# ORNL/DDStore

Measured on NVIDIA H100. Metric: batch_fetch_GBps, higher is better.
Workload: dtype u8

## Files before the change

### ddstore_b200/csrc/kernels.cu

```cuda
#include <cuda_runtime.h>
#include <stdint.h>
#include <stdio.h>
#include <stdlib.h>
#include <string.h>

#include <algorithm>
#include <atomic>
#include <type_traits>

#include "kernels.h"

namespace {

thread_local char g_cuda_err[512] = "";
std::atomic<unsigned long long> g_launches{0};

#define CUDA_TRY(expr)                                                                                   \
    do {                                                                                                 \
        cudaError_t e__ = (expr);                                                                        \
        if (e__ != cudaSuccess) {                                                                        \
            snprintf(g_cuda_err, sizeof(g_cuda_err), "%s failed: %s (%s:%d)", #expr, cudaGetErrorString(e__), \
                     __FILE__, __LINE__);                                                                \
            return (int)e__ ? (int)e__ : -1;                                                             \
        }                                                                                                \
// ... 1004 lines not shown
    return T;
}

struct PieceDesc {
    int64_t dpos;
    uint32_t n, pack;
};

__device__ __forceinline__ void spin_until_done(const unsigned int *ovl, unsigned int q, unsigned long long *status,
                                                unsigned long long tag, int64_t nreq) {
    const uint64_t t0 = globaltimer_ns();
    while ((int)(ld_acquire_u32(&ovl[4 + (q & 3u)]) - q) < 0) {
        __nanosleep(100);
        if (globaltimer_ns() - t0 > 4000000000ull) {
            report(status, tag, nreq, DDSK_CODE_WATCHDOG);
            __trap();
        }
    }
}

template <bool FIXED, int NW, int S, int CH, int PCAP, bool CVT = false, bool NORM = false, bool PAD = false, bool PUT = false>
__global__ void __launch_bounds__(NW * 32, 1) dds_gather_kernel(const __grid_constant__ GatherArgs a,
                                                                const __grid_constant__ CvtParam<CVT> c) {
    static_assert(CVT || !NORM, "a normalising launch is a converting one");
    static_assert(FIXED || !PAD, "a padded batch is a fixed-stride walk");
    static_assert(!PUT || (!CVT && !PAD), "a put writes raw rows");
    constexpr int STAGE = CH + 32;
    constexpr bool PUSH = FIXED && !CVT && !PAD && !PUT;
    extern __shared__ __align__(128) unsigned char smem_dyn[];
    __shared__ __align__(8) uint64_t full_bar[NW][S];
    __shared__ __align__(16) PieceDesc desc[NW][S][32];
    __shared__ int64_t wtot[PCAP > 0 ? NW : 1];
    __shared__ int64_t push_rbase[PUSH ? DDSK_MAX_RANKS + 1 : 1];
    __shared__ uint64_t push_win[PUSH ? DDSK_MAX_RANKS : 1];

    const int lane = threadIdx.x & 31;
    const int warp = threadIdx.x >> 5;
    const int64_t gwarp = (int64_t)blockIdx.x * NW + warp;
    const int64_t nwarps = (int64_t)gridDim.x * NW;

    if (lane == 0) {
#pragma unroll
        for (int s = 0; s < S; s++) mbar_init(smem_u32(&full_bar[warp][s]), 1);
        fence_mbar_init();
    }
    uint32_t lut_s = 0;
    if constexpr (CVT) {
        lut_s = smem_u32(smem_dyn) + (uint32_t)(NW * S * STAGE + (PCAP ? PCAP * 12 + 16 : 0));
        for (int i = threadIdx.x; i < c.lut_bytes / 4; i += NW * 32) sts32(lut_s + 4u * (uint32_t)i, c.lut[i]);
        __syncthreads();
    }
    int code0 = 0;
    if constexpr (CVT) code0 = c.code[0];
    if (a.dbg && threadIdx.x == 0) a.dbg[blockIdx.x * 4 + 0] = globaltimer_ns();
    if (a.overlap && !a.wait1_valid) {
        asm volatile("griddepcontrol.wait;" ::: "memory");
        asm volatile("griddepcontrol.launch_dependents;" ::: "memory");
    } else {
        asm volatile("griddepcontrol.launch_dependents;" ::: "memory");
        if (!a.skip_wait) asm volatile("griddepcontrol.wait;" ::: "memory");
    }
    bool gate_open = !(a.overlap && a.wait2_valid);
    auto pass_gate = [&]() {
        if (!gate_open) {
            if (lane == 0) spin_until_done(a.ovl, a.seq - 2u, a.status, a.status_tag, a.nreq);
            __syncwarp();
            gate_open = true;
        }
    };

    ChunkWalker<FIXED, CH, PCAP, CVT, PAD, PUT> w;
    if (!FIXED) {
        if constexpr (PCAP > 0) {
            w.pv.src_s = smem_u32(smem_dyn) + (uint32_t)(NW * S * STAGE);
            w.pv.dst_s = w.pv.src_s + (uint32_t)PCAP * 8u;
            const bool writer = blockIdx.x == 0;
            if (writer) pass_gate();
            w.T = plan_in_smem<NW, PCAP, CVT, NORM, PUT>(a, w.pv, wtot, warp, lane, writer, code0);
        } else {
            w.pv.src = a.req_src;
            w.pv.dst = a.req_dst;
            w.pv.seg_tab = a.seg_tab;
            if (a.wait_plan) {
                const bool need_gate = !gate_open;
                unsigned long long pw = 0;
                const uint64_t t0 = globaltimer_ns();
                while (true) {
                    bool ok = true;
                    if (lane == 0) {
                        pw = ld_acquire_u64(&a.plan_word[a.seq & 3u]);
                        ok = (pw >> 40) == (unsigned long long)a.plan_tiles;
                    } else if (lane == 1 && need_gate) {
                        ok = (int)(ld_acquire_u32(&a.ovl[4 + ((a.seq - 2u) & 3u)]) - (a.seq - 2u)) >= 0;
                    }
                    if (__all_sync(0xffffffffu, ok)) break;
                    __nanosleep(100);
                    if (globaltimer_ns() - t0 > 4000000000ull) {
                        report(a.status, a.status_tag, a.nreq, DDSK_CODE_WATCHDOG);
                        __trap();
                    }
                }
                gate_open = true;
                w.T = (int64_t)(__shfl_sync(0xffffffffu, pw, 0) & 0xFFFFFFFFFFull);
            } else {
                w.T = __ldcg(&a.req_dst[a.nreq]);
            }
        }
    }

    const bool push = PUSH && a.push != nullptr;
    if (FIXED && push) {
        const ddsk_push_t *ps = a.push;
        const int P = ps->nranks, me = ps->me, par = (int)(a.push_step & 1ull);
        if (blockIdx.x == 0 && threadIdx.x == 0) {
            unsigned long long *hdr = (unsigned long long *)ps->win[me];
            *(volatile unsigned long long *)&hdr[1 + par] = (unsigned long long)a.push_nreq;
            __threadfence_system();
            st_release_sys_u64(&hdr[0], a.push_step);
        }
        const uint64_t t0 = globaltimer_ns();
        for (int r0 = 0; r0 < P; r0 += 32) {
            const int r = r0 + lane;
            while (r < P && ld_acquire_sys_u64((const unsigned long long *)ps->win[r]) < a.push_step) {
                __nanosleep(200);
                if (globaltimer_ns() - t0 > 30000000000ull) {
                    report(a.status, a.status_tag, a.nreq, DDSK_CODE_WATCHDOG);
                    __trap();
                }
            }
        }
        __syncwarp();
        if (warp == 0) {
            int64_t n = 0;
            for (int r0 = 0; r0 < P; r0 += 32) {
                const int r = r0 + lane;
                int64_t mine_n = 0;
                if (r < P) {
                    push_win[r] = (uint64_t)ps->win[r];
                    mine_n = ld_relaxed_sys_s64((const int64_t *)ps->win[r] + 1 + par);
                }
                const int64_t incl = warp_incl_scan(mine_n, lane);
                if (r < P) push_rbase[r] = n + incl - mine_n;
                n += __shfl_sync(0xffffffffu, incl, 31);
            }
            if (lane == 0) push_rbase[P] = n;
        }
        __syncthreads();
        w.push_n = P;
        w.push_me = me;
        w.push_par = par;
        w.push_rbase = push_rbase;
        w.push_win = push_win;
        w.push_idx_off = ps->idx_off[par];
    }
    if (a.dbg && threadIdx.x == 0) a.dbg[blockIdx.x * 4 + 1] = globaltimer_ns();
    bool dbg_first = a.dbg != nullptr && warp == 0;
    w.gwarp = gwarp;
    w.nwarps = nwarps;
    w.static_claims = a.tickets == nullptr;
    w.gate_ok = gate_open;
    if constexpr (PAD) w.nb = a.pad_slot;
    else w.nb = (FIXED && a.count <= a.var.lenlist[a.var.nranks - 1]) ? a.count * a.var.row_bytes : 0;
    w.nreq = (FIXED && push) ? push_rbase[w.push_n] : a.nreq;
    if (FIXED) w.T = w.nb * w.nreq;
    bool over = w.T > a.dst_cap;
    const int64_t push_dst_off = (FIXED && push) ? a.push->dst_off[w.push_par] : 0;
    const bool multi = !FIXED && a.plan.nvars > 1;
    int64_t vbase[DDSK_MAX_MULTI + 1];
#pragma unroll
    for (int v = 0; v <= DDSK_MAX_MULTI; v++) vbase[v] = INT64_MAX;
    if (multi) {
        over = false;
#pragma unroll
        for (int v = 0; v < DDSK_MAX_MULTI; v++)
            if (v < a.plan.nvars) vbase[v] = w.pv.d((int64_t)v * a.plan.per_var);
#pragma unroll
        for (int v = 0; v < DDSK_MAX_MULTI; v++)
            if (v < a.plan.nvars) {
                const int64_t endv = v + 1 < a.plan.nvars ? vbase[v + 1] : w.T;
                over |= endv - vbase[v] > a.mcap[v];
            }
        if (PCAP > 0) over |= w.T > 0xFFFFFFFFll;
        if constexpr (CVT) {
            w.valign = true;
#pragma unroll
            for (int v = 0; v < DDSK_MAX_MULTI; v++) w.vb[v] = vbase[v];
        }
    }
    auto dst_of = [&](int64_t dpos) -> char * {
        if (FIXED && push) {
            int p = 0;
            for (int k = 1; k < w.push_n; k++)
                if (dpos >= push_rbase[k] * w.nb) p = k;
            return (char *)push_win[p] + push_dst_off + (dpos - push_rbase[p] * w.nb);
        }
        if (!multi) return a.dst + dpos;
        int64_t b = vbase[0];
        char *d = a.mdst[0];
#pragma unroll
        for (int k = 1; k < DDSK_MAX_MULTI; k++)
            if (dpos >= vbase[k]) {
                b = vbase[k];
                d = a.mdst[k];
            }
        return d + (dpos - b);
    };
    auto out_of = [&](int64_t dpos, int &code, uint32_t &lut) -> char * {
        if constexpr (CVT) {
            if (!multi) {
// ... 158 lines not shown
        }
        }
        bulk_commit();
        __syncwarp();
        consumed++;
    }
    if (PUT || a.overlap || (FIXED && push)) {
        bulk_wait_all<0>();
        fence_proxy_async_global();
    } else {
        bulk_wait_read<0>();
    }
    __syncwarp();
    pass_gate();
    if (multi) {
        for (int64_t i = gwarp * 32 + lane; i < a.nreq + a.plan.nvars; i += nwarps * 32) {
            const int v = (int)(i / (a.plan.per_var + 1));
            const int64_t j = i - (int64_t)v * (a.plan.per_var + 1);
            if (v < a.plan.nvars && a.moffsets[v]) {
                const int64_t basev = w.pv.d((int64_t)v * a.plan.per_var);
                int64_t e = (v * a.plan.per_var + j == a.nreq) ? w.T : w.pv.d((int64_t)v * a.plan.per_var + j);
                if constexpr (CVT) a.moffsets[v][j] = cvt_scale<NORM>(e - basev, c.code[v]);
                else a.moffsets[v][j] = e - basev;
            }
        }
        if constexpr (CVT) {
            if (gwarp == 0 && lane == 0 && a.total_out) {
                int64_t t = 0;
#pragma unroll
                for (int v = 0; v < DDSK_MAX_MULTI; v++)
                    if (v < a.plan.nvars) t += cvt_scale<NORM>((v + 1 < a.plan.nvars ? vbase[v + 1] : w.T) - vbase[v], c.code[v]);
                *a.total_out = t;
            }
        }
    }
    if constexpr (PAD) {
        if (a.pad_lengths || w.nb == 0) {
            for (int64_t i = gwarp * 32 + lane; i < a.nreq; i += nwarps * 32) {
                uint64_t src;
                int64_t payload;
                pad_lookup(a, i, src, payload);
                if (a.pad_lengths) a.pad_lengths[i] = payload / a.var.row_bytes;
            }
        }
    }
    if (FIXED && a.offsets_out && !push) {
        if constexpr (CVT) {
            for (int64_t i = gwarp * 32 + lane; i <= a.nreq; i += nwarps * 32) a.offsets_out[i] = cvt_scale<NORM>(i * w.nb, code0);
        } else {
            for (int64_t i = gwarp * 32 + lane; i <= a.nreq; i += nwarps * 32) a.offsets_out[i] = i * w.nb;
        }
    }

    if (a.dbg && lane == 0) atomicMax(&a.dbg[blockIdx.x * 4 + 3], (unsigned long long)globaltimer_ns());
    if (a.overlap) {
        if (lane == 0) {
            __threadfence();
            const unsigned int slot = a.seq & 3u;
            const unsigned int done = atomicAdd(&a.ovl[slot], 1u);
            if (done == (unsigned int)(nwarps - 1)) {
                a.ovl[slot] = 0;
                a.ovl[8 + slot] = 0;
                if (a.wait_plan) a.plan_word[slot] = 0;
                if (a.wait1_valid) spin_until_done(a.ovl, a.seq - 1u, a.status, a.status_tag, a.nreq);
                __threadfence();
                st_release_u32(&a.ovl[4 + slot], a.seq);
            }
        }
    } else if (lane == 0) {
        if (FIXED && push) __threadfence_system(); else __threadfence();
        unsigned int done = atomicAdd(&a.counters[1], 1u);
        if (done == (unsigned int)(nwarps - 1)) {
            a.counters[0] = 0;
            a.counters[1] = 0;
            __threadfence();
            if (FIXED && push) {
                const ddsk_push_t *ps = a.push;
                for (int r = 0; r < ps->nranks; r++)
                    st_release_sys_u64((unsigned long long *)ps->win[r] + 8 + ps->me, a.push_step);
                const unsigned long long *hdr = (const unsigned long long *)ps->win[ps->me];
                const uint64_t t0 = globaltimer_ns();
                for (int r = 0; r < ps->nranks; r++)
                    while (ld_acquire_sys_u64(&hdr[8 + r]) < a.push_step) {
                        __nanosleep(200);
                        if (globaltimer_ns() - t0 > 30000000000ull) {
                            report(a.status, a.status_tag, a.nreq, DDSK_CODE_WATCHDOG);
                            __trap();
                        }
                    }
                const unsigned long long st = *(volatile const unsigned long long *)&hdr[3];
                if (st != DDSK_STATUS_OK) atomicMin(a.status, st | a.status_tag);
            }
            if (a.host_mirror) {
                a.host_mirror[0] = *(volatile unsigned long long *)a.status;
                a.host_mirror[1] = (unsigned long long)w.T;
                __threadfence_system();
            }
        }
    }
}

__global__ void __launch_bounds__(256) dds_small_get_kernel(const __grid_constant__ ddsk_var_t var, int64_t start, int64_t count,
                                                            char *__restrict__ dst, int64_t dst_cap,
                                                            volatile unsigned long long *flag, unsigned long long ticket) {
    uint64_t src = 0;
    const int code = dev_locate(var, start, count, &src);
    const int64_t n = code ? 0 : count * var.row_bytes;
    unsigned long long st = DDSK_STATUS_OK;
    if (code) st = (unsigned long long)code;
    else if (n > dst_cap) st = ((unsigned long long)1 << 8) | DDSK_CODE_CAPACITY;
    if (st == DDSK_STATUS_OK && n > 0) {
        const char *s = (const char *)src;
        if ((((uint64_t)s | (uint64_t)dst | (uint64_t)n) & 15u) == 0) {
            const uint4 *s4 = (const uint4 *)s;
            uint4 *d4 = (uint4 *)dst;
            for (int64_t i = threadIdx.x; i < (n >> 4); i += blockDim.x) d4[i] = s4[i];
        } else if ((((uint64_t)s | (uint64_t)dst | (uint64_t)n) & 3u) == 0) {
            const uint32_t *s1 = (const uint32_t *)s;
            uint32_t *d1 = (uint32_t *)dst;
            for (int64_t i = threadIdx.x; i < (n >> 2); i += blockDim.x) d1[i] = s1[i];
        } else {
            for (int64_t i = threadIdx.x; i < n; i += blockDim.x) dst[i] = s[i];
        }
    }
    __threadfence_system();
// ... 215 lines not shown
                for (int64_t i = threadIdx.x; i < (n >> 2); i += blockDim.x) ((uint32_t *)dp)[i] = __ldcg((const unsigned int *)sp + i);
            } else {
                for (int64_t i = threadIdx.x; i < n; i += blockDim.x) dp[i] = __ldcg(sp + i);
            }
            __threadfence_system();
        }
        __syncthreads();
        if (threadIdx.x == 0) *(volatile unsigned long long *)&mb->resp = (q << 8) | st;
        served = q;
    }
}

__global__ void dds_touch_kernel(const uint4 *__restrict__ p, size_t n, unsigned int *sink) {
    unsigned int acc = 0;
    for (size_t i = (size_t)blockIdx.x * blockDim.x + threadIdx.x; i < n; i += (size_t)gridDim.x * blockDim.x) {
        const uint4 v = p[i];
        acc ^= v.x ^ v.y ^ v.z ^ v.w;
    }
    if (acc == 0x9E3779B9u && sink) *sink = acc;
}

__global__ void dds_occupy_kernel(unsigned long long ns, int smem_bytes) {
    extern __shared__ unsigned char occ_smem[];
    if ((int)threadIdx.x < smem_bytes) occ_smem[threadIdx.x] = (unsigned char)threadIdx.x;
    const uint64_t t0 = globaltimer_ns();
    while (globaltimer_ns() - t0 < ns) __nanosleep(1000);
    if ((int)threadIdx.x < smem_bytes && occ_smem[threadIdx.x] == 255 && ns == 0) printf("");
}

struct Geometry {
    int nw, stages, ch, pcap;
};
constexpr Geometry kGeoms[] = {{8, 4, 4096, 0}, {8, 6, 4096, 0}, {16, 3, 4096, 0}, {4, 4, 8192, 0}, {12, 4, 4096, 0}, {4, 6, 4096, 0},
                               {6, 4, 4096, 0},
                               {12, 3, 4096, 0}};
constexpr int kNumGeoms = (int)(sizeof(kGeoms) / sizeof(kGeoms[0]));
constexpr Geometry kGeomsS[] = {{12, 3, 4096, 4096}, {12, 3, 3072, 8192}, {16, 3, 2048, 8192}, {16, 3, 3072, 4096}, {8, 4, 4096, 4096}};
constexpr int kNumGeomsS = (int)(sizeof(kGeomsS) / sizeof(kGeomsS[0]));
constexpr int64_t kPlanSmemMax = 8192;
int64_t g_plan_smem_default = 1024;

constexpr int kGeomLarge = 4, kGeomSmall = 2, kGeomVar = 4;

int g_geom_fixed_env = -1;
int g_geom_var_env = -1;
int g_geom_s_env = -1;
int g_min_seg_var = 4, g_min_seg_s = 2;
bool g_geom_init = false;
int g_sms = 0;
int g_ctas_per_sm = 1;
int g_pdl = 1;
unsigned long long *g_dbg = nullptr;
constexpr size_t kDbgRegion = 4096 + 8;
int g_l2_persist = 1;
int g_smem_plan = 1;

int pick_geometry() {
    if (g_geom_init) return 0;
    int dev = 0;
    CUDA_TRY(cudaGetDevice(&dev));
    CUDA_TRY(cudaDeviceGetAttribute(&g_sms, cudaDevAttrMultiProcessorCount, dev));
    if (const char *e = getenv("DDS_GATHER_GEOM")) g_geom_fixed_env = atoi(e);
    if (g_geom_fixed_env >= kNumGeoms) g_geom_fixed_env = -1;
    g_geom_var_env = g_geom_fixed_env;
    if (const char *e = getenv("DDS_GATHER_GEOM_VAR")) g_geom_var_env = atoi(e);
    if (g_geom_var_env >= kNumGeoms) g_geom_var_env = -1;
    if (const char *e = getenv("DDS_GATHER_GEOM_S")) g_geom_s_env = atoi(e);
    if (g_geom_s_env >= kNumGeomsS) g_geom_s_env = -1;
    if (const char *e = getenv("DDS_VAR_MINSEG")) g_min_seg_var = atoi(e) > 0 ? atoi(e) : 4;
    if (const char *e = getenv("DDS_S_MINSEG")) g_min_seg_s = atoi(e) > 0 ? atoi(e) : 2;
    if (const char *e = getenv("DDS_GATHER_CTAS_PER_SM")) g_ctas_per_sm = atoi(e) > 0 ? atoi(e) : 1;
    if (const char *e = getenv("DDS_PDL")) g_pdl = atoi(e) != 0;
    if (const char *e = getenv("DDS_SMEM_PLAN")) g_smem_plan = atoi(e);
    if (const char *e = getenv("DDS_SMEM_PLAN_MAX")) g_plan_smem_default = atoll(e);
    if (const char *e = getenv("DDS_L2_PERSIST")) g_l2_persist = atoi(e);
    if (const char *e = getenv("DDS_DEBUG_TIMING"))
        if (atoi(e)) {
            CUDA_TRY(cudaMalloc((void **)&g_dbg, 2 * kDbgRegion * 8));
            CUDA_TRY(cudaMemset(g_dbg, 0, 2 * kDbgRegion * 8));
        }
    g_geom_init = true;
    return 0;
}

int geometry_for(bool fixed, int64_t request_bytes) {
    if (fixed) {
        if (g_geom_fixed_env >= 0) return g_geom_fixed_env;
        return request_bytes < 2048 ? kGeomSmall : kGeomLarge;
    }
    return g_geom_var_env >= 0 ? g_geom_var_env : kGeomVar;
}
int geometry_s_for(int64_t nreq) {
    if (nreq > kPlanSmemMax || nreq > g_plan_smem_default) return -1;
    if (g_geom_s_env >= 0 && kGeomsS[g_geom_s_env].pcap >= nreq) return g_geom_s_env;
    return nreq <= 4096 ? 0 : 1;
}

constexpr int smem_bytes_of(int nw, int s, int ch, int pcap) { return nw * s * (ch + 32) + (pcap ? pcap * 12 + 16 : 0); }
int static_smem_of(int nw, int s) { return nw * s * (8 + 32 * 16) + 16 * 8 + 64; }
int ctas_per_sm_for(int nw, int s, int ch, int pcap) {
    int per_sm = g_ctas_per_sm;
    while (per_sm > 1 && per_sm * (smem_bytes_of(nw, s, ch, pcap) + static_smem_of(nw, s) + 1024) > 227 * 1024) per_sm--;
    return per_sm;
}

bool cvt_has_norm(const ddsk_cvt_t *cvt) {
    for (int v = 0; v < DDSK_MAX_MULTI; v++)
        if (DDSK_CVT_IS_NORM(cvt->code[v])) return true;
    return false;
}

template <bool FIXED, int NW, int S, int CH, int PCAP, bool CVT = false, bool NORM = false, bool PAD = false, bool PUT = false>
int launch_gather_t(const GatherArgs &args_in, cudaStream_t stream, const ddsk_cvt_t *cvt = nullptr) {
    const int smem = smem_bytes_of(NW, S, CH, PCAP) + (CVT ? cvt->lut_bytes : 0);
    static std::atomic<unsigned long long> configured{0};
    auto kern = dds_gather_kernel<FIXED, NW, S, CH, PCAP, CVT, NORM, PAD, PUT>;
    int dev = 0;
    CUDA_TRY(cudaGetDevice(&dev));
    if (CVT) {
        if (dev >= 64 || !(configured.load() & (1ull << dev))) {
            cudaFuncAttributes fa;
            int optin = 0;
            CUDA_TRY(cudaFuncGetAttributes(&fa, kern));
            CUDA_TRY(cudaDeviceGetAttribute(&optin, cudaDevAttrMaxSharedMemoryPerBlockOptin, dev));
            const int most = std::min(smem_bytes_of(NW, S, CH, PCAP) + DDSK_MAX_MULTI * 1024, optin - (int)fa.sharedSizeBytes);
            CUDA_TRY(cudaFuncSetAttribute(kern, cudaFuncAttributeMaxDynamicSharedMemorySize, most));
            if (dev < 64) configured.fetch_or(1ull << dev);
        }
    } else if (dev >= 64 || !(configured.load() & (1ull << dev))) {
        CUDA_TRY(cudaFuncSetAttribute(kern, cudaFuncAttributeMaxDynamicSharedMemorySize, smem));
        if (dev < 64) configured.fetch_or(1ull << dev);
    }
    const int per_sm = ctas_per_sm_for(NW, S, CH, PCAP);
    GatherArgs args = args_in;
    args.dbg = g_dbg ? g_dbg + (size_t)(args.overlap ? (args.seq & 1u) : 0u) * kDbgRegion : nullptr;
    cudaLaunchConfig_t cfg = {};
    cfg.gridDim = dim3((unsigned)(g_sms * per_sm));
    cfg.blockDim = dim3(NW * 32);
    cfg.dynamicSmemBytes = smem;
    cfg.stream = stream;
    cudaLaunchAttribute attr[1];
    attr[0].id = cudaLaunchAttributeProgrammaticStreamSerialization;
    attr[0].val.programmaticStreamSerializationAllowed = g_pdl ? 1 : 0;
    cfg.attrs = attr;
    cfg.numAttrs = 1;
    if constexpr (CVT) {
        CUDA_TRY(cudaLaunchKernelEx(&cfg, kern, args, *cvt));
    } else {
        CUDA_TRY(cudaLaunchKernelEx(&cfg, kern, args, NoCvt{0}));
    }
    g_launches++;
    return 0;
}

template <int NW, int S, int CH, int PCAP>
bool cvt_s_fits_t(int lut_bytes) {
    cudaFuncAttributes fa;
    int dev = 0, optin = 0;
    if (cudaGetDevice(&dev) != cudaSuccess || cudaFuncGetAttributes(&fa, dds_gather_kernel<false, NW, S, CH, PCAP, true>) != cudaSuccess ||
        cudaDeviceGetAttribute(&optin, cudaDevAttrMaxSharedMemoryPerBlockOptin, dev) != cudaSuccess) {
        (void)cudaGetLastError();
        return false;
    }
    return smem_bytes_of(NW, S, CH, PCAP) + lut_bytes + (int)fa.sharedSizeBytes <= optin;
}

thread_local const void *g_l2_base = nullptr;
thread_local size_t g_l2_bytes = 0;

template <typename... KArgs, typename... Args>
int launch_pdl(void (*kern)(KArgs...), dim3 grid, dim3 block, cudaStream_t st, Args... args) {
    cudaLaunchConfig_t cfg = {};
    cfg.gridDim = grid;
    cfg.blockDim = block;
    cfg.dynamicSmemBytes = 0;
    cfg.stream = st;
    cudaLaunchAttribute attr[2];
    attr[0].id = cudaLaunchAttributeProgrammaticStreamSerialization;
    attr[0].val.programmaticStreamSerializationAllowed = g_pdl ? 1 : 0;
    cfg.attrs = attr;
    cfg.numAttrs = 1;
    if (g_l2_base && g_l2_bytes && g_l2_persist) {
        attr[1].id = cudaLaunchAttributeAccessPolicyWindow;
        attr[1].val.accessPolicyWindow.base_ptr = const_cast<void *>(g_l2_base);
        attr[1].val.accessPolicyWindow.num_bytes = g_l2_bytes;
        attr[1].val.accessPolicyWindow.hitRatio = 1.0f;
        attr[1].val.accessPolicyWindow.hitProp = cudaAccessPropertyPersisting;
        attr[1].val.accessPolicyWindow.missProp = cudaAccessPropertyStreaming;
        cfg.numAttrs = 2;
    }
    g_l2_base = nullptr;
    g_l2_bytes = 0;
    CUDA_TRY(cudaLaunchKernelEx(&cfg, kern, args...));
    g_launches++;
    return 0;
}

template <bool FIXED>
int launch_gather(const GatherArgs &args, cudaStream_t stream, const ddsk_cvt_t *cvt, bool put = false) {
    if (put) return launch_gather_t<FIXED, 12, 4, 4096, 0, false, false, false, true>(args, stream);
    if (cvt) return cvt_has_norm(cvt) ? launch_gather_t<FIXED, 12, 4, 4096, 0, true, true>(args, stream, cvt)
                                      : launch_gather_t<FIXED, 12, 4, 4096, 0, true>(args, stream, cvt);
    const int64_t request_bytes = args.count < ((int64_t)1 << 20) ? args.count * args.var.row_bytes : INT64_MAX;
    switch (geometry_for(FIXED, FIXED ? request_bytes : 0)) {
    case 1: return launch_gather_t<FIXED, 8, 6, 4096, 0>(args, stream);
    case 2: return launch_gather_t<FIXED, 16, 3, 4096, 0>(args, stream);
    case 3: return launch_gather_t<FIXED, 4, 4, 8192, 0>(args, stream);
    case 4: return launch_gather_t<FIXED, 12, 4, 4096, 0>(args, stream);
    case 5: return launch_gather_t<FIXED, 4, 6, 4096, 0>(args, stream);
    case 6: return launch_gather_t<FIXED, 6, 4, 4096, 0>(args, stream);
    case 7: return launch_gather_t<FIXED, 12, 3, 4096, 0>(args, stream);
    default: return launch_gather_t<FIXED, 8, 4, 4096, 0>(args, stream);
    }
}
int launch_gather_s(int g, const GatherArgs &args, cudaStream_t stream, const ddsk_cvt_t *cvt, bool put) {
    if (put)
        return g == 1 ? launch_gather_t<false, 12, 3, 3072, 8192, false, false, false, true>(args, stream)
                      : launch_gather_t<false, 12, 3, 4096, 4096, false, false, false, true>(args, stream);
    if (cvt && cvt_has_norm(cvt))
        return g == 1 ? launch_gather_t<false, 12, 3, 3072, 8192, true, true>(args, stream, cvt)
                      : launch_gather_t<false, 12, 3, 4096, 4096, true, true>(args, stream, cvt);
    if (cvt) return g == 1 ? launch_gather_t<false, 12, 3, 3072, 8192, true>(args, stream, cvt)
                           : launch_gather_t<false, 12, 3, 4096, 4096, true>(args, stream, cvt);
    switch (g) {
    case 1: return launch_gather_t<false, 12, 3, 3072, 8192>(args, stream);
    case 2: return launch_gather_t<false, 16, 3, 2048, 8192>(args, stream);
    case 3: return launch_gather_t<false, 16, 3, 3072, 4096>(args, stream);
    case 4: return launch_gather_t<false, 8, 4, 4096, 4096>(args, stream);
    default: return launch_gather_t<false, 12, 3, 4096, 4096>(args, stream);
    }
}

int select_s(int64_t nreq, int64_t cap, const ddsk_cvt_t *cvt, bool put = false) {
    if (!g_smem_plan || cap >= ((int64_t)1 << 32)) return -1;
    if (!cvt && !put) return geometry_s_for(nreq);
    if (nreq > kPlanSmemMax || nreq > g_plan_smem_default) return -1;
    if (put) return nreq <= 4096 ? 0 : 1;
    if (nreq <= 4096) return cvt_s_fits_t<12, 3, 4096, 4096>(cvt->lut_bytes) ? 0 : -1;
    return cvt_s_fits_t<12, 3, 3072, 8192>(cvt->lut_bytes) ? 1 : -1;
}

void fill_overlap(GatherArgs &a, const ddsk_scratch_t *scr, int flags) {
    a.overlap = (flags & DDSK_F_OVERLAP) ? 1 : 0;
    a.skip_wait = (flags & DDSK_F_SKIP_WAIT) ? 1 : 0;
    a.wait1_valid = (flags & DDSK_F_PREV1) ? 1 : 0;
    a.wait2_valid = (flags & DDSK_F_PREV2) ? 1 : 0;
    a.seq = scr->ovl_seq;
    a.ovl = scr->ovl;
    a.tickets = a.overlap ? nullptr : scr->counters;
}

}

extern "C" {

const char *ddsk_last_cuda_error(void) { return g_cuda_err; }
// ... 51 lines not shown
    if (int rc = pick_geometry()) return rc;
    GatherArgs a;
    memset(&a, 0, sizeof(a));
    a.var = *var;
    a.count = count;
    a.nreq = nreq;
    a.dst = nullptr;
    a.dst_cap = INT64_MAX;
    a.status = scr->status;
    a.status_tag = scr->status_tag;
    a.counters = scr->counters;
    a.tickets = scr->counters;
    a.min_seg_chunks = 1;
    a.push = push_dev;
    if (nreq > 0)
        CUDA_TRY(cudaMemcpyAsync(push_host->win[push_host->me] + push_host->idx_off[step & 1ull], starts_dev, (size_t)nreq * 8,
                                 cudaMemcpyDeviceToDevice, st));
    a.push_nreq = nreq;
    a.push_step = step;
    return launch_gather<true>(a, st, nullptr);
}

int ddsk_gather_padded(const ddsk_var_t *var, const ddsk_index_t *index, int64_t nreq, int64_t max_rows, uint64_t pad_bits,
                       int pad_log2, int64_t *lengths, void *dst_dev, const ddsk_scratch_t *scr, int flags,
                       const ddsk_cvt_t *cvt, void *stream) {
    cudaStream_t st = (cudaStream_t)stream;
    if (flags & DDSK_F_RESET) CUDA_TRY(cudaMemsetAsync(scr->status, 0xFF, sizeof(unsigned long long), st));
    if (nreq <= 0) return 0;
    if (int rc = pick_geometry()) return rc;
    GatherArgs a;
    memset(&a, 0, sizeof(a));
    a.var = *var;
    a.plan.starts = index->starts;
    a.plan.counts = index->counts;
    a.plan.ids = index->sample_ids;
    a.plan.tab = (const longlong2 *)index->table;
    a.plan.nsamples = index->nsamples;
    a.count = max_rows;
    a.nreq = nreq;
    a.dst = (char *)dst_dev;
    a.pad_slot = max_rows * var->row_bytes;
    a.dst_cap = nreq * a.pad_slot;
    a.pad_bits = pad_bits;
    a.pad_log2 = pad_log2;
    a.pad_in_log2 = cvt ? cvt_in_log2<true>(cvt->code[0]) : 0;
    a.pad_out_log2 = cvt ? cvt_out_log2<true>(cvt->code[0]) : 0;
    a.pad_lengths = lengths;
    a.status = scr->status;
    a.status_tag = scr->status_tag;
    a.counters = scr->counters;
    a.min_seg_chunks = 1;
    fill_overlap(a, scr, flags);
    a.host_mirror = (flags & DDSK_F_MIRROR) ? scr->host_mirror : nullptr;
    if (!cvt) return launch_gather_t<true, 12, 4, 4096, 0, false, false, true>(a, st);
    return cvt_has_norm(cvt) ? launch_gather_t<true, 12, 4, 4096, 0, true, true, true>(a, st, cvt)
                             : launch_gather_t<true, 12, 4, 4096, 0, true, false, true>(a, st, cvt);
}

static int plan_and_gather(const ddsk_var_t *var, const PlanSrc &p, int64_t nreq, int64_t cap_total, GatherArgs &a,
                           int64_t *offsets_dev_or_null, ddsk_scratch_t *scr, int flags, const ddsk_cvt_t *cvt,
                           cudaStream_t st) {
    a.nreq = nreq;
    a.status = scr->status;
    a.status_tag = scr->status_tag;
    a.counters = scr->counters;
    a.host_mirror = (flags & DDSK_F_MIRROR) ? scr->host_mirror : nullptr;
    a.plan = p;
    a.total_out = scr->total;
    const bool put = (flags & DDSK_F_PUT) != 0;
    const int gs = select_s(nreq, cap_total, cvt, put);
    if (gs >= 0) {
        a.offsets_out = offsets_dev_or_null;
        a.min_seg_chunks = g_min_seg_s;
        fill_overlap(a, scr, flags);
        if (a.overlap) a.tickets = scr->ovl + 8 + (a.seq & 3u);
        return launch_gather_s(gs, a, st, cvt, put);
    }
    if (nreq > scr->cap_req || cap_total / SEG_GRAIN + 2 > scr->seg_cap) {
        snprintf(g_cuda_err, sizeof(g_cuda_err), "ddsk_gather_var: scratch too small (%lld requests > %lld, or %lld segments > %lld)",
                 (long long)nreq, (long long)scr->cap_req, (long long)(cap_total / SEG_GRAIN + 2), (long long)scr->seg_cap);
        return -2;
    }
    PlanProto pr;
    memset(&pr, 0, sizeof(pr));
    if (flags & DDSK_F_OVERLAP) {
        pr.dbg = g_dbg ? g_dbg + (size_t)(scr->ovl_seq & 1u) * kDbgRegion : nullptr;
        pr.ovl = scr->ovl;
        pr.plan_word = scr->plan_word;
        pr.seq = scr->ovl_seq;
        pr.skip_wait = (flags & DDSK_F_SKIP_WAIT) ? 1 : 0;
        pr.wait2_valid = (flags & DDSK_F_PREV2) ? 1 : 0;
        pr.wait4_valid = (flags & DDSK_F_PREV4) ? 1 : 0;
    }
    const int tiles = (int)((nreq + PLAN_TILE - 1) / PLAN_TILE);
    scr->plan_tag = (scr->plan_tag + 1) & 0x3FFFFFu;
    if (p.ids && (p.tab || p.mtab[0])) {
        g_l2_base = p.tab ? (const void *)p.tab : (const void *)p.mtab[0];
        g_l2_bytes = (size_t)(p.tab ? p.nsamples : p.mnsamples[0]) * 16;
    }
    if (int rc = launch_pdl(put ? dds_plan_kernel<true> : dds_plan_kernel<false>, dim3(tiles), dim3(PLAN_THREADS), st, *var, p, nreq, scr->req_src, scr->req_dst,
                            (unsigned long long *)scr->tile_sums, scr->plan_tag, offsets_dev_or_null, scr->seg_tab, scr->seg_cap,
                            scr->status, scr->status_tag, pr, cvt && p.nvars <= 1 ? (int)cvt->code[0] : 0))
        return rc;
    a.req_src = scr->req_src;
    a.req_dst = scr->req_dst;
    a.seg_tab = scr->seg_tab;
// ... 155 lines not shown
```

### ddstore_b200/cython/pyddstore.pyx

```
"""pyddstore -- Cython binding with the reference module's name and Python surface
(/root/reference/src/pyddstore.pyx:58-131: PyDDStore(comm, method=0) with add / get / epoch_begin /
epoch_end / free / init / update), bound to the C++ class in include/ddstore_b200.hpp, which is a thin
wrapper over the C-ABI (include/ddstore_b200.h) of libddstore_b200.so.

Differences from the reference binding, all at the edges:
  * `comm` is anything ddstore_b200.comm.as_dds_comm accepts (an mpi4py-style communicator, a
    torch.distributed adapter, ShmComm, None) -- MPI is not required;
  * arrays may also be CUDA tensors / __cuda_array_interface__ objects (then nothing touches the host);
  * `get_batch` fetches a whole batch in one kernel launch.
"""
from libcpp.string cimport string
from libcpp cimport bool as cbool
from libc.stdint cimport uint64_t

import numpy as np

from ddstore_b200.comm import as_dds_comm
from ddstore_b200.store import _Buf, _conversion, _dtype_name, _i64, _norm_tables, _pad_bits, _ptr

cdef extern from *:
    """
    static void dds_translate_exception() {
        try { throw; }
        catch (const std::invalid_argument &e) { PyErr_SetString(PyExc_ValueError, e.what()); }
        catch (const std::out_of_range &e) { PyErr_SetString(PyExc_KeyError, e.what()); }
        catch (const std::exception &e) { PyErr_SetString(PyExc_RuntimeError, e.what()); }
    }
    """
    void dds_translate_exception()

cdef extern from "ddstore_b200.h":
    ctypedef struct dds_comm_t:
        pass

cdef extern from "ddstore_b200.hpp" nogil:
    cdef cppclass DDStore:
        DDStore(int method, dds_comm_t* comm, int device) except +dds_translate_exception
        void add[T](string name, T* buffer, long nrows, int disp) except +dds_translate_exception
        void add_device[T](string name, const T* buffer, long nrows, int disp) except +dds_translate_exception
        void get[T](string name, long start, long count, T* buffer) except +dds_translate_exception
        void get_device[T](string name, long start, long count, T* buffer) except +dds_translate_exception
        long get_batch[T](string name, const long* starts, const long* counts, long fixed_count, long nreq, T* dst,
                          long cap, long* offsets, cbool on_device, void* stream) except +dds_translate_exception
        long get_batch_convert(string name, const long* starts, const long* counts, long fixed_count, long nreq,
                               void* dst, long cap, int code, const void* lut, long* offsets, cbool idx_on_device,
                               void* stream) except +dds_translate_exception
        long get_batch_padded_convert(string name, const long* starts, const long* counts, long nreq, int itemsize,
                                      int code, const void* lut, long max_rows, uint64_t pad_bits, void* dst, long cap,
                                      long* lengths, cbool idx_on_device, void* stream) except +dds_translate_exception
        void set_normalization(string name, const float* mean, const float* std, long nchan, long inner,
                               cbool tables_on_device) except +dds_translate_exception
        long put_batch[T](string name, const long* starts, const long* counts, long fixed_count, long nreq, const T* src,
                          long src_bytes, cbool idx_on_device, void* stream) except +dds_translate_exception
        void epoch_begin() except +dds_translate_exception
        void epoch_end() except +dds_translate_exception
        void free() except +dds_translate_exception
        void init(string name, long nrows, int disp, int itemsize) except +dds_translate_exception
        void update[T](string name, T* buffer, long nrows, long offset) except +dds_translate_exception
        int rank()
        int size()


cdef class PyDDStore:
    cdef DDStore* c_ddstore
    cdef object _comm

    def __cinit__(self, comm=None, int method=0, device=None):
        self._comm = as_dds_comm(comm)
        cdef size_t h = <size_t> self._comm.handle
        cdef int dev = -1 if device is None else int(device)
        with nogil:
            self.c_ddstore = new DDStore(method, <dds_comm_t*> h, dev)

    def __dealloc__(self):
        if self.c_ddstore != NULL:
            del self.c_ddstore
            self.c_ddstore = NULL

    @property
    def rank(self):
        return self.c_ddstore.rank()

    @property
    def size(self):
        return self.c_ddstore.size()

# ... 241 lines not shown
```

### ddstore_b200/store.py

```python
import ctypes as C

import numpy as np

from . import _capi
from .comm import as_dds_comm

_NP_OK = {np.dtype(np.int32), np.dtype(np.int64), np.dtype(np.uint8), np.dtype(np.float32),
          np.dtype(np.float64), np.dtype(np.bool_)}
_TORCH_OK = {"torch.int32", "torch.int64", "torch.uint8", "torch.float32", "torch.float64", "torch.bool"}
_TORCH_HALF = {"torch.bfloat16", "torch.float16"}

_CVT_CODES = {("float32", "bfloat16"): _capi.CVT_F32_BF16, ("float32", "float16"): _capi.CVT_F32_F16,
              ("float64", "float32"): _capi.CVT_F64_F32, ("uint8", "bfloat16"): _capi.CVT_U8_LUT16,
              ("uint8", "float16"): _capi.CVT_U8_LUT16, ("uint8", "float32"): _capi.CVT_U8_LUT32}
_NORM_CODES = {("float32", "float32"): _capi.CVT_NORM_F32_F32, ("float32", "bfloat16"): _capi.CVT_NORM_F32_BF16,
               ("float32", "float16"): _capi.CVT_NORM_F32_F16, ("float64", "float32"): _capi.CVT_NORM_F64_F32,
               ("uint8", "float32"): _capi.CVT_NORM_U8_F32, ("uint8", "bfloat16"): _capi.CVT_NORM_U8_BF16,
               ("uint8", "float16"): _capi.CVT_NORM_U8_F16}
_U8_NORM = (_capi.CVT_NORM_U8_F32, _capi.CVT_NORM_U8_BF16, _capi.CVT_NORM_U8_F16)
_default_luts = {}


def _dtype_name(dt):
    s = str(dt)
# ... 76 lines not shown
        if isinstance(value, float) and not value.is_integer():
            raise ValueError(f"pad_value {value!r} is not an integer ({dtype})")
        iv, info = int(value), torch.iinfo(dtype)
        if not info.min <= iv <= info.max:
            raise ValueError(f"pad_value {value!r} is outside the range of {dtype}")
        t = torch.tensor([iv], dtype=dtype)
    n = t.element_size()
    return int(t.view(getattr(torch, _INT_VIEW[n])).item()) & ((1 << (8 * n)) - 1)


def _lut_bits(t):
    import torch
    t = t.detach().reshape(-1).cpu().contiguous()
    return t.view(torch.int16 if t.element_size() == 2 else torch.int32).numpy().copy()


class _Buf:

    def __init__(self, arr, writable=False, half_ok=False):
        self.keep = arr
        if isinstance(arr, np.ndarray):
            assert arr.flags.c_contiguous
            if arr.dtype not in _NP_OK:
                raise NotImplementedError
            self.ptr, self.on_device = arr.ctypes.data, 0
            self.shape, self.itemsize, self.size = arr.shape, arr.dtype.itemsize, arr.size
        elif hasattr(arr, "data_ptr") and hasattr(arr, "element_size"):
            assert arr.is_contiguous()
            if str(arr.dtype) not in _TORCH_OK and not (half_ok and str(arr.dtype) in _TORCH_HALF):
                raise NotImplementedError
            self.ptr, self.on_device = arr.data_ptr(), 1 if arr.is_cuda else 0
            self.shape, self.itemsize, self.size = tuple(arr.shape), arr.element_size(), arr.numel()
        elif hasattr(arr, "__cuda_array_interface__"):
            cai = arr.__cuda_array_interface__
            if cai.get("strides") is not None:
                raise ValueError("device array must be C-contiguous")
            dt = np.dtype(cai["typestr"])
            if dt not in _NP_OK:
                raise NotImplementedError
            self.ptr, self.on_device = cai["data"][0], 1
            self.shape, self.itemsize = tuple(cai["shape"]), dt.itemsize
            self.size = int(np.prod(self.shape, dtype=np.int64))
        else:
            raise TypeError(f"unsupported array type {type(arr).__name__}")
        self.nbytes = self.size * self.itemsize


class _DevMem:

    def __init__(self, ptr, nbytes):
        self.__cuda_array_interface__ = {"shape": (int(nbytes),), "typestr": "|u1", "data": (int(ptr), False), "version": 2}


def _i64(x):
    return np.ascontiguousarray(x, dtype=np.int64)


class PyDDStore:
    def __init__(self, comm=None, method=0, device=None):
        self._L = _capi.lib()
        self._comm = as_dds_comm(comm)
        self._h = self._L.dds_create(self._comm.handle, -1 if device is None else int(device), int(method))
        if not self._h:
            raise RuntimeError(_capi.last_error())
        self.rank, self.size = self._L.dds_rank(self._h), self._L.dds_size(self._h)
        self._itemsize = {}
        self._cname = {}
        self._rowbytes = {}
        self.last_bad_index = -1

    def add(self, name, arr):
        b = _Buf(arr)
        nrows = b.shape[0]
        disp = b.size // b.shape[0] if b.shape[0] else int(np.prod(b.shape[1:], dtype=np.int64))
        _capi.raise_for(self._L.dds_add(self._h, name.encode(), b.ptr, nrows, disp, b.itemsize, b.on_device))

    def get(self, name, arr, start=0):
        cn = self._cname.get(name)
        if cn is None:
            cn = self._cname[name] = name.encode()
        if type(arr) is np.ndarray:
            assert arr.flags.c_contiguous
            if arr.dtype not in _NP_OK:
                raise NotImplementedError
            rc = self._L.dds_get(self._h, cn, int(start), arr.shape[0], arr.dtype.itemsize, arr.ctypes.data, 0)
        else:
            b = _Buf(arr, writable=True)
            rc = self._L.dds_get(self._h, cn, int(start), b.shape[0], b.itemsize, b.ptr, b.on_device)
        if rc:
            _capi.raise_for(rc)

    def epoch_begin(self):
        _capi.raise_for(self._L.dds_epoch_begin(self._h))

    def epoch_end(self):
        _capi.raise_for(self._L.dds_epoch_end(self._h))

    def free(self):
        if self._h:
            self._itemsize.clear()
            _capi.raise_for(self._L.dds_free(self._h))

    def init(self, name, nrows, disp, itemsize=1):
        _capi.raise_for(self._L.dds_init(self._h, name.encode(), int(nrows), int(disp), int(itemsize)))

    def update(self, name, arr, offset, stream=None, wait=True):
        b = _Buf(arr)
        if wait:
            rc = self._L.dds_update(self._h, name.encode(), b.ptr, b.shape[0], int(offset), b.itemsize, b.on_device)
        else:
            rc = self._L.dds_update_async(self._h, name.encode(), b.ptr, b.shape[0], int(offset), b.itemsize,
                                          b.on_device, self._stream_arg(stream))
        _capi.raise_for(rc)

    def ingest(self, name, arr, offset):
        b = _Buf(arr)
        if b.on_device:
            raise ValueError("ingest takes host arrays (use update for device arrays)")
        _capi.raise_for(self._L.dds_ingest(self._h, name.encode(), b.ptr, b.shape[0], int(offset), b.itemsize))

    def ingest_wait(self):
        _capi.raise_for(self._L.dds_ingest_wait(self._h))

    def get_batch(self, name, starts, counts=None, out=None, count=None, offsets=None, stream=None, wait=True,
                  overlap=False, src_dtype=None, lut=None, normalize=False, pad_rows=None, pad_value=0, lengths=None):
        if out is None:
            raise ValueError("get_batch needs an `out` buffer (like get(), it never allocates)")
        if pad_rows is not None:
            if counts is None:
                raise ValueError("pad_rows needs counts (there is no fixed-count padded batch)")
            if count is not None or offsets is not None:
                raise ValueError("a padded batch takes neither `count` nor `offsets`")
        cv = lut_keep = None
        if normalize and src_dtype is None:
            raise ValueError("normalize=True needs src_dtype")
        if src_dtype is not None:
            cv, lut_keep = _conversion(src_dtype, getattr(out, "dtype", None), lut, normalize)
        else:
            itemsize = self._itemsize.get(name)
            if itemsize is None:
                itemsize = self._itemsize[name] = self.query(name)["itemsize"]
        ob = _Buf(out, writable=True, half_ok=cv is not None or pad_rows is not None)
        s_dev = hasattr(starts, "data_ptr") and getattr(starts, "is_cuda", False)
        if s_dev:
            nreq = starts.numel()
            sp = starts.data_ptr()
            cp = counts.data_ptr() if counts is not None else None
            keep = (starts, counts)
        else:
            sa = _i64(starts)
            nreq = sa.size
            sp = sa.ctypes.data
            ca = _i64(counts) if counts is not None else None
            cp = ca.ctypes.data if ca is not None else None
            keep = (sa, ca)
        flags = (_capi.IDX_ON_DEVICE if s_dev else 0) | (_capi.DST_ON_DEVICE if ob.on_device else 0)
        if not wait:
            flags |= _capi.NO_SYNC | (_capi.OVERLAP if overlap else 0)
        if pad_rows is not None:
            return self._padded(name, False, sp, cp, nreq, out, ob, cv, pad_rows, pad_value, lengths, flags, stream,
                                (keep, lut_keep))
        op = None
        if offsets is not None:
            fb = _Buf(offsets, writable=True)
            if fb.on_device != ob.on_device or fb.itemsize != 8 or fb.size < nreq + 1:
                raise ValueError("offsets must be int64[len(starts)+1] with the same residency as out")
            op = fb.ptr
        total, bad = C.c_int64(0), C.c_int64(-1)
        if cv is None:
            rc = self._L.dds_get_batch(self._h, name.encode(), sp, cp, 1 if count is None else int(count), nreq,
                                       itemsize, ob.ptr, ob.nbytes, op, flags,
                                       self._stream_arg(stream), C.byref(total), C.byref(bad))
        else:
            rc = self._L.dds_get_batch_convert(self._h, name.encode(), sp, cp, 1 if count is None else int(count), nreq,
                                               ob.ptr, ob.nbytes, op, flags, self._stream_arg(stream), C.byref(cv),
                                               C.byref(total), C.byref(bad))
        del keep, lut_keep
        self.last_bad_index = bad.value
        _capi.raise_for(rc)
        return total.value
# ... 260 lines not shown
```

Before: 1432.

## Add small-grid gather path, per-CTA completion counting, and Cython fast get_batch

Adds a small-geometry gather kernel (6 warps, 4 stages) launched on a grid sized to the batch when the total transfer fits in one wave, so tiny batches do not pay for a full persistent grid. Completion counting moves from one atomic per warp to one per CTA after a __syncthreads, cutting global atomics at kernel end. A Cython entry point lets fixed-count device-index batches skip the ctypes and Python argument-handling path. Debug timing is also limited to the first 1024 blocks. The risks are the extra block barrier, reduced parallelism for mid-size batches, and an import path that depends on finding the compiled .so.

```diff
diff --git a/ddstore_b200/csrc/kernels.cu b/ddstore_b200/csrc/kernels.cu
--- a/ddstore_b200/csrc/kernels.cu
+++ b/ddstore_b200/csrc/kernels.cu
@@ -1080,7 +1080,8 @@
     }
     int code0 = 0;
     if constexpr (CVT) code0 = c.code[0];
-    if (a.dbg && threadIdx.x == 0) a.dbg[blockIdx.x * 4 + 0] = globaltimer_ns();
+    const bool dbg = a.dbg != nullptr && blockIdx.x < 1024;
+    if (dbg && threadIdx.x == 0) a.dbg[blockIdx.x * 4 + 0] = globaltimer_ns();
     if (a.overlap && !a.wait1_valid) {
         asm volatile("griddepcontrol.wait;" ::: "memory");
         asm volatile("griddepcontrol.launch_dependents;" ::: "memory");
@@ -1181,8 +1182,8 @@
         w.push_win = push_win;
         w.push_idx_off = ps->idx_off[par];
     }
-    if (a.dbg && threadIdx.x == 0) a.dbg[blockIdx.x * 4 + 1] = globaltimer_ns();
-    bool dbg_first = a.dbg != nullptr && warp == 0;
+    if (dbg && threadIdx.x == 0) a.dbg[blockIdx.x * 4 + 1] = globaltimer_ns();
+    bool dbg_first = dbg && warp == 0;
     w.gwarp = gwarp;
     w.nwarps = nwarps;
     w.static_claims = a.tickets == nullptr;
@@ -1447,13 +1448,14 @@
         }
     }
 
-    if (a.dbg && lane == 0) atomicMax(&a.dbg[blockIdx.x * 4 + 3], (unsigned long long)globaltimer_ns());
+    if (dbg && lane == 0) atomicMax(&a.dbg[blockIdx.x * 4 + 3], (unsigned long long)globaltimer_ns());
+    __syncthreads();
     if (a.overlap) {
-        if (lane == 0) {
+        if (threadIdx.x == 0) {
             __threadfence();
             const unsigned int slot = a.seq & 3u;
             const unsigned int done = atomicAdd(&a.ovl[slot], 1u);
-            if (done == (unsigned int)(nwarps - 1)) {
+            if (done == gridDim.x - 1) {
                 a.ovl[slot] = 0;
                 a.ovl[8 + slot] = 0;
                 if (a.wait_plan) a.plan_word[slot] = 0;
@@ -1462,10 +1464,10 @@
                 st_release_u32(&a.ovl[4 + slot], a.seq);
             }
         }
-    } else if (lane == 0) {
+    } else if (threadIdx.x == 0) {
         if (FIXED && push) __threadfence_system(); else __threadfence();
         unsigned int done = atomicAdd(&a.counters[1], 1u);
-        if (done == (unsigned int)(nwarps - 1)) {
+        if (done == gridDim.x - 1) {
             a.counters[0] = 0;
             a.counters[1] = 0;
             __threadfence();
@@ -1787,6 +1789,8 @@
 int g_pdl = 1;
 unsigned long long *g_dbg = nullptr;
 constexpr size_t kDbgRegion = 4096 + 8;
+constexpr int kSmallNW = 6, kSmallS = 4, kSmallCH = 4096;
+int g_small_grid = 2;
 int g_l2_persist = 1;
 int g_smem_plan = 1;
 
@@ -1809,6 +1813,7 @@
     if (const char *e = getenv("DDS_SMEM_PLAN")) g_smem_plan = atoi(e);
     if (const char *e = getenv("DDS_SMEM_PLAN_MAX")) g_plan_smem_default = atoll(e);
     if (const char *e = getenv("DDS_L2_PERSIST")) g_l2_persist = atoi(e);
+    if (const char *e = getenv("DDS_SMALL_GRID")) g_small_grid = atoi(e);
     if (const char *e = getenv("DDS_DEBUG_TIMING"))
         if (atoi(e)) {
             CUDA_TRY(cudaMalloc((void **)&g_dbg, 2 * kDbgRegion * 8));
@@ -1839,6 +1844,15 @@
     return per_sm;
 }
 
+int small_grid_for(int64_t T, int sms, int stages) {
+    if (stages <= 0) return 0;
+    const int64_t per_cta = (int64_t)kSmallNW * kSmallCH * stages;
+    const int64_t wave = (int64_t)sms * ((227 * 1024) / (smem_bytes_of(kSmallNW, kSmallS, kSmallCH, 0) +
+                                                          static_smem_of(kSmallNW, kSmallS) + 1024));
+    const int64_t ctas = T <= 0 ? 1 : T / per_cta + (T % per_cta != 0);
+    return ctas <= wave ? (int)ctas : 0;
+}
+
 bool cvt_has_norm(const ddsk_cvt_t *cvt) {
     for (int v = 0; v < DDSK_MAX_MULTI; v++)
         if (DDSK_CVT_IS_NORM(cvt->code[v])) return true;
@@ -1846,7 +1860,7 @@
 }
 
 template <bool FIXED, int NW, int S, int CH, int PCAP, bool CVT = false, bool NORM = false, bool PAD = false, bool PUT = false>
-int launch_gather_t(const GatherArgs &args_in, cudaStream_t stream, const ddsk_cvt_t *cvt = nullptr) {
+int launch_gather_t(const GatherArgs &args_in, cudaStream_t stream, const ddsk_cvt_t *cvt = nullptr, int grid = 0) {
     const int smem = smem_bytes_of(NW, S, CH, PCAP) + (CVT ? cvt->lut_bytes : 0);
     static std::atomic<unsigned long long> configured{0};
     auto kern = dds_gather_kernel<FIXED, NW, S, CH, PCAP, CVT, NORM, PAD, PUT>;
@@ -1870,7 +1884,7 @@
     GatherArgs args = args_in;
     args.dbg = g_dbg ? g_dbg + (size_t)(args.overlap ? (args.seq & 1u) : 0u) * kDbgRegion : nullptr;
     cudaLaunchConfig_t cfg = {};
-    cfg.gridDim = dim3((unsigned)(g_sms * per_sm));
+    cfg.gridDim = dim3((unsigned)(grid > 0 ? grid : g_sms * per_sm));
     cfg.blockDim = dim3(NW * 32);
     cfg.dynamicSmemBytes = smem;
     cfg.stream = stream;
@@ -1934,9 +1948,17 @@
 template <bool FIXED>
 int launch_gather(const GatherArgs &args, cudaStream_t stream, const ddsk_cvt_t *cvt, bool put = false) {
     if (put) return launch_gather_t<FIXED, 12, 4, 4096, 0, false, false, false, true>(args, stream);
+    const int64_t request_bytes = args.count < ((int64_t)1 << 20) ? args.count * args.var.row_bytes : INT64_MAX;
+    if constexpr (FIXED) {
+        const int64_t T = request_bytes <= 0 ? 0 : args.nreq > INT64_MAX / request_bytes ? INT64_MAX : args.nreq * request_bytes;
+        const int g = args.push ? 0 : small_grid_for(T, g_sms, g_small_grid);
+        if (g > 0 && cvt)
+            return cvt_has_norm(cvt) ? launch_gather_t<true, kSmallNW, kSmallS, kSmallCH, 0, true, true>(args, stream, cvt, g)
+                                     : launch_gather_t<true, kSmallNW, kSmallS, kSmallCH, 0, true>(args, stream, cvt, g);
+        if (g > 0 && g_geom_fixed_env < 0) return launch_gather_t<true, kSmallNW, kSmallS, kSmallCH, 0>(args, stream, nullptr, g);
+    }
     if (cvt) return cvt_has_norm(cvt) ? launch_gather_t<FIXED, 12, 4, 4096, 0, true, true>(args, stream, cvt)
                                       : launch_gather_t<FIXED, 12, 4, 4096, 0, true>(args, stream, cvt);
-    const int64_t request_bytes = args.count < ((int64_t)1 << 20) ? args.count * args.var.row_bytes : INT64_MAX;
     switch (geometry_for(FIXED, FIXED ? request_bytes : 0)) {
     case 1: return launch_gather_t<FIXED, 8, 6, 4096, 0>(args, stream);
     case 2: return launch_gather_t<FIXED, 16, 3, 4096, 0>(args, stream);
@@ -2094,6 +2116,11 @@
     a.min_seg_chunks = 1;
     fill_overlap(a, scr, flags);
     a.host_mirror = (flags & DDSK_F_MIRROR) ? scr->host_mirror : nullptr;
+    if (const int g = small_grid_for(a.dst_cap, g_sms, g_small_grid)) {
+        if (!cvt) return launch_gather_t<true, kSmallNW, kSmallS, kSmallCH, 0, false, false, true>(a, st, nullptr, g);
+        return cvt_has_norm(cvt) ? launch_gather_t<true, kSmallNW, kSmallS, kSmallCH, 0, true, true, true>(a, st, cvt, g)
+                                 : launch_gather_t<true, kSmallNW, kSmallS, kSmallCH, 0, true, false, true>(a, st, cvt, g);
+    }
     if (!cvt) return launch_gather_t<true, 12, 4, 4096, 0, false, false, true>(a, st);
     return cvt_has_norm(cvt) ? launch_gather_t<true, 12, 4, 4096, 0, true, true, true>(a, st, cvt)
                              : launch_gather_t<true, 12, 4, 4096, 0, true, false, true>(a, st, cvt);
diff --git a/ddstore_b200/cython/pyddstore.pyx b/ddstore_b200/cython/pyddstore.pyx
--- a/ddstore_b200/cython/pyddstore.pyx
+++ b/ddstore_b200/cython/pyddstore.pyx
@@ -11,7 +11,7 @@
 """
 from libcpp.string cimport string
 from libcpp cimport bool as cbool
-from libc.stdint cimport uint64_t
+from libc.stdint cimport int64_t, uint64_t
 
 import numpy as np
 
@@ -32,6 +32,23 @@
 cdef extern from "ddstore_b200.h":
     ctypedef struct dds_comm_t:
         pass
+    ctypedef struct dds_store_t:
+        pass
+    int dds_get_batch(dds_store_t *s, const char *name, const int64_t *starts, const int64_t *counts,
+                      int64_t fixed_count, int64_t nreq, int itemsize, void *dst, int64_t dst_capacity,
+                      int64_t *dst_offsets, unsigned flags, void *cuda_stream, int64_t *total_bytes,
+                      int64_t *bad_index) nogil
+
+
+def get_batch_fixed(size_t store, const char *name, size_t starts, int64_t count, int64_t nreq, int itemsize,
+                    size_t dst, int64_t cap, size_t offsets, unsigned flags, size_t stream):
+    """dds_get_batch of a fixed-count batch, called straight from Python: the per-call path of ddstore_b200.PyDDStore's
+    get_batch for device indices into a device buffer (a queue of small batches is bound by what one call costs the
+    host). Arguments are the C-ABI's, pointers as integers (0 = NULL). -> (return code, packed bytes, bad index)"""
+    cdef int64_t total = 0, bad = -1
+    cdef int rc = dds_get_batch(<dds_store_t *>store, name, <const int64_t *>starts, NULL, count, nreq, itemsize,
+                                <void *>dst, cap, <int64_t *>offsets, flags, <void *>stream, &total, &bad)
+    return rc, total, bad
 
 cdef extern from "ddstore_b200.hpp" nogil:
     cdef cppclass DDStore:
diff --git a/ddstore_b200/store.py b/ddstore_b200/store.py
--- a/ddstore_b200/store.py
+++ b/ddstore_b200/store.py
@@ -152,6 +152,33 @@
         self.__cuda_array_interface__ = {"shape": (int(nbytes),), "typestr": "|u1", "data": (int(ptr), False), "version": 2}
 
 
+_fast_get = None
+
+
+def _fast_entry():
+    global _fast_get
+    if _fast_get is None:
+        _fast_get = False
+        import glob
+        import importlib.util
+        import os
+        import sys
+        for path in glob.glob(os.path.join(os.path.dirname(os.path.abspath(__file__)), "cython", "pyddstore*.so")):
+            mod = sys.modules.get("pyddstore")
+            if mod is None:
+                try:
+                    spec = importlib.util.spec_from_file_location("pyddstore", path)
+                    mod = importlib.util.module_from_spec(spec)
+                    sys.modules["pyddstore"] = mod
+                    spec.loader.exec_module(mod)
+                except ImportError:
+                    sys.modules.pop("pyddstore", None)
+                    break
+            _fast_get = getattr(mod, "get_batch_fixed", False)
+            break
+    return _fast_get or None
+
+
 def _i64(x):
     return np.ascontiguousarray(x, dtype=np.int64)
 
@@ -226,6 +253,23 @@
                   overlap=False, src_dtype=None, lut=None, normalize=False, pad_rows=None, pad_value=0, lengths=None):
         if out is None:
             raise ValueError("get_batch needs an `out` buffer (like get(), it never allocates)")
+        fast = _fast_entry()
+        if (fast is not None and counts is None and offsets is None and pad_rows is None and src_dtype is None
+                and not normalize and self._h and getattr(starts, "is_cuda", False) and hasattr(starts, "data_ptr")
+                and getattr(out, "is_cuda", False) and hasattr(out, "element_size") and out.is_contiguous()
+                and str(out.dtype) in _TORCH_OK):
+            itemsize = self._itemsize.get(name)
+            if itemsize is None:
+                itemsize = self._itemsize[name] = self.query(name)["itemsize"]
+            flags = _capi.IDX_ON_DEVICE | _capi.DST_ON_DEVICE
+            if not wait:
+                flags |= _capi.NO_SYNC | (_capi.OVERLAP if overlap else 0)
+            sh = 0 if stream is None else (int(stream) or 1)
+            rc, total, bad = fast(self._h, name.encode(), starts.data_ptr(), 1 if count is None else int(count),
+                                  starts.numel(), itemsize, out.data_ptr(), out.numel() * out.element_size(), 0, flags, sh)
+            self.last_bad_index = bad
+            _capi.raise_for(rc)
+            return total
         if pad_rows is not None:
             if counts is None:
                 raise ValueError("pad_rows needs counts (there is no fixed-count padded batch)")
```

New measurement: 1433 (median of 6 runs). No clear change (+0.0%).
